# SegoleneMartin/transductive-CLIP

Measured on AMD Instinct MI355X. Metric: transductive tasks/sec (75-query EM-Dirichlet), higher is better.
Workload: dtype f32

## Files before the change

### include/tclip.h

```cpp
#ifndef TCLIP_H
#define TCLIP_H

#include <stddef.h>
#include <stdint.h>

#ifdef __cplusplus
extern "C" {
#endif

#define TCLIP_ABI_VERSION 5

enum {
    TCLIP_OK = 0,
    TCLIP_ERR_ARG = 1,
    TCLIP_ERR_WORKSPACE = 2,
    TCLIP_ERR_HIP = 3,
    TCLIP_ERR_INDEX = 4
};

typedef struct tclip_problem {
    int32_t n_batches;
    int32_t tasks_per_batch;
    int32_t n_query;
    int32_t n_class;
// ... 53 lines not shown
int tclip_em_gaussian_run(const tclip_problem* p, const float* x_q, float temperature, float* u, float* v, float* w,
                          int32_t* preds, void* workspace, size_t workspace_bytes, void* stream);

int tclip_em_gaussian_cov_run(const tclip_problem* p, const float* x_q, float* u, float* v, float* w, float* s,
                              int32_t* preds, void* workspace, size_t workspace_bytes, void* stream);

size_t tclip_hard_kmeans_workspace_bytes(const tclip_problem* p);
int tclip_hard_kmeans_run(const tclip_problem* p, const float* x_q, float* u, float* w, int32_t* preds,
                          float* criterions, void* workspace, size_t workspace_bytes, void* stream);

int tclip_kl_kmeans_run(const tclip_problem* p, const float* x_q, float* u, float* w, int32_t* preds,
                        float* criterions, void* workspace, size_t workspace_bytes, void* stream);

size_t tclip_bdcspn_workspace_bytes(const tclip_problem* p);
int tclip_bdcspn_run(const tclip_problem* p, const float* x_q, const float* x_s, const int64_t* y_s, float temp,
                     int32_t norm_type, float* prototypes, float* u, int32_t* preds, void* workspace,
                     size_t workspace_bytes, void* stream);

size_t tclip_paddle_workspace_bytes(const tclip_problem* p);
int tclip_paddle_run(const tclip_problem* p, const float* x_q, const float* x_s, const int64_t* y_s, float lambd,
                     float* u, float* v, float* w, int32_t* preds, void* workspace, size_t workspace_bytes,
                     void* stream);

#define TCLIP_TIM_SHANNON 0
#define TCLIP_TIM_ALPHA 1
typedef struct tclip_tim_params {
    double lr;
    float temp;
    float alpha_value;
    float loss_weights[3];
    int32_t entropies[3];
} tclip_tim_params;
size_t tclip_alpha_tim_workspace_bytes(const tclip_problem* p);
int tclip_alpha_tim_run(const tclip_problem* p, const tclip_tim_params* prm, const float* x_q, const float* x_s,
                        const int64_t* y_s, float* weights, float* logits_q, int32_t* preds, float* criterions,
                        void* workspace, size_t workspace_bytes, void* stream);

size_t tclip_laplacian_shot_workspace_bytes(const tclip_problem* p);
int tclip_laplacian_shot_run(const tclip_problem* p, const float* x_q, const float* x_s, const int64_t* y_s, int32_t knn,
                             double lmd, int32_t norm_type, float* unary, int32_t* neighbours, int32_t* preds_iter,
                             double* energies, void* workspace, size_t workspace_bytes, void* stream);

int tclip_argmax_rows(const float* x, int64_t n_rows, int32_t n_class, int32_t* labels, void* stream);

int tclip_probability_features(const float* visual, const float* text, int64_t n_rows, int32_t dim, int32_t n_class,
                               float temperature, float* out, void* stream);

int tclip_profile_enable(int on);
int tclip_profile_collect(double* mm_busy_ms, double* mm_launch_ms_sum, int64_t* mm_launches,
                          int64_t* element_updates);
int tclip_profile_last_kernels(double* busy_ms, double* launch_ms_sum, int64_t* launches, int64_t* element_updates);
int tclip_profile_last_split_sorts(int64_t* wave_iterations, int64_t* sorts);
int tclip_debug_set_split_keep_placement(int32_t on);

int tclip_debug_set_probe_chunks(int32_t chunks);

int tclip_debug_set_dead_head(int32_t iterations);

int tclip_debug_set_rowset_min_rows(int32_t rows);

int tclip_debug_set_mm_split(int32_t mode);

int tclip_debug_set_fixed_k_kernels(int32_t on);

int tclip_debug_set_kmeans_tile(int32_t mode);

int tclip_selftest_primitives(uint64_t* mismatches);

#ifdef __cplusplus
}
#endif
#endif
```

### transductive-clip_amd/csrc/tclip_kernels.hip

```cpp
#include <hip/hip_runtime.h>
#include <stdint.h>
#include <stdio.h>
#include <stdlib.h>
#include <string.h>

#include <algorithm>
#include <mutex>
#include <utility>
#include <vector>

#include "../../include/tclip.h"
#include "tclip_device.h"
#include "tclip_pk.h"
#include "tclip_selftest_inputs.h"

namespace tclip {

constexpr int kG64MinK = 897;

__global__ void k_log_features(const float* __restrict__ x, float* __restrict__ out, size_t n, int32_t* __restrict__ nonfinite) {
    bool bad = false;
    for (size_t i = (size_t)blockIdx.x * blockDim.x + threadIdx.x; i < n; i += (size_t)gridDim.x * blockDim.x) {
        const float v = log_f32(x[i] + kEpsF);
        out[i] = v;
// ... 262 lines not shown
        }
    }
    for (; i < Q; ++i) {
        const float fv = ft[(size_t)i * K];
#pragma unroll
        for (int j = 0; j < kMstatsRows; j++) a0[j] += term(j, ut[(size_t)i * K + j], fv);
    }
#pragma unroll
    for (int j = 0; j < kMstatsRows; j++) {
        const size_t row = (size_t)t * K + k0 + j;
        if (!live[row]) continue;
        float s = a0[j];
        s += a1[j];
        s += a2[j];
        s += a3[j];
        const float c = cs[row];
        if (kCov) {
            y[row * K + d] = c / (s < kEpsF ? kEpsF : s);
        } else if (paddle == 2) {
            y[row * K + d] = s / c;
        } else if (sup && paddle) {
            y[row * K + d] = (s + sup[row * K + d]) / (c + cnt[row]);
        } else if (sup) {
            const float w = 1.0f / (cnt[row] + c);
            y[row * K + d] = w * (sup[row * K + d] + s);
        } else {
            y[row * K + d] = s / (c < kEpsF ? kEpsF : c);
        }
    }
}

__device__ __forceinline__ int lanes_below_mask(unsigned long long m, int lane) { return __popcll(m & ((1ull << lane) - 1ull)); }

__global__ void k_build_rows(const uint8_t* __restrict__ live, const int32_t* __restrict__ cache_len, int n_rows,
                             int n_checks, int32_t* __restrict__ dead_rows, int32_t* __restrict__ live_rows,
                             int32_t* __restrict__ n_dead, int32_t* __restrict__ n_live) {
    const int i = blockIdx.x * blockDim.x + threadIdx.x;
    const bool in = i < n_rows;
    const bool alive = in && live[i];
    const bool need = in && !alive && n_checks > 0 && cache_len[i] < n_checks;
    const unsigned long long ml = __ballot(alive), md = __ballot(need);
    const int lane64 = threadIdx.x & 63;
    int base_l = 0, base_d = 0;
    if (lane64 == 0) {
        if (ml) base_l = atomicAdd(n_live, __popcll(ml));
        if (md) base_d = atomicAdd(n_dead, __popcll(md));
    }
    base_l = __shfl(base_l, 0, 64);
    base_d = __shfl(base_d, 0, 64);
    if (alive) live_rows[base_l + lanes_below_mask(ml, lane64)] = i;
    if (need) dead_rows[base_d + lanes_below_mask(md, lane64)] = i;
}

struct MMArgs {
    float* alpha;
    float* beta_dead;
    const float* y;
    const uint8_t* live;
    int32_t* cache_len;
    double* cache;
    double* rowpart;
    const int32_t* rows;
    const int32_t* n_rows;
    const int32_t* stop;
    unsigned long long* work_counter;
    int32_t* next_rows;
    int32_t* next_count;
    int K, rows_per_batch, chunk, l0, l1, has_check, n_checks;
    int keep_placement;
};

constexpr int kYRegsMaxE = 16;
template <int E, int G>
__device__ __forceinline__ int elem_of(int e, int lane) {
    if constexpr (G == 64) return (lane >> 5) * (E * 32) + e * 32 + (lane & 31);
    else return e * G + lane;
}
template <int E, int G>
__host__ __device__ constexpr int full_registers(int K) {
    if constexpr (G == 64) return K > E * 32 ? (K - E * 32) / 32 : 0;
    else return K / G;
}

template <int E, int G = kGroup, int kRegsMaxE = kYRegsMaxE>
struct RowY {
    static constexpr bool kInRegs = E <= kRegsMaxE;
    float r[kInRegs ? E : 1];
    const float* g;
    int lane, K, n_full;
    __device__ __forceinline__ void load(const float* row_y, int lane_, int K_) {
        g = row_y; lane = lane_; K = K_; n_full = full_registers<E, G>(K_);
        if (kInRegs) {
#pragma unroll
            for (int e = 0; e < (kInRegs ? E : 1); e++) {
                const int d = elem_of<E, G>(e, lane);
                r[e] = d < K ? (g ? g[d] : -10.0f) : 0.0f;
            }
        }
    }
    __device__ __forceinline__ void fetch_all(float (&out)[E]) const {
        if (!g) {
#pragma unroll
            for (int e = 0; e < E; e++) out[e] = -10.0f;
            return;
        }
        if constexpr (G == 64) {
            const float* base = g;
            asm volatile("" : "+s"(base));
            const __amdgpu_buffer_rsrc_t rsrc = __builtin_amdgcn_make_buffer_rsrc((void*)base, 0, K * 4, 0x00020000);
            int voff = elem_of<E, G>(0, lane) * 4;
            asm volatile("" : "+v"(voff));
#pragma unroll
            for (int e = 0; e < E; e++) out[e] = __builtin_bit_cast(float, __builtin_amdgcn_raw_buffer_load_b32(rsrc, voff + e * 128, 0, 0));
        } else {
#pragma unroll
            for (int e = 0; e < E; e++) out[e] = get(e);
        }
    }
    __device__ __forceinline__ float get(int e) const {
        if (kInRegs) return r[kInRegs ? e : 0];
// ... 447 lines not shown
        for (int w = 1; w < W; w++) at += j >= before[w] ? 64 * E * R - (before[w] - before[w - 1]) : 0;
        const float v = j < n_big ? queue[at] : 8.0f;
        const float r = lgamma_big_dense(v);
        if (j < n_big) queue[at] = r;
    }
    if (wave == (W - (turn % W) + 1) % W && lane64 < kGroups * R)
        ctl->psi[turn & 1][lane64] = digamma_pos_f32(ctl->rowsum[turn & 1][lane64], tab);
    __syncthreads();
    if (base[R] == 0) {
#pragma unroll
        for (int r = 0; r < R; r++)
            if (active[r])
                mm_apply_updates_small<E, G>(beta[r], yv[r], K, lane, ctl->psi[turn & 1][r * kGroups + (threadIdx.x / G)], tab,
                                             measure, num[r], den[r]);
        return;
    }
#pragma unroll
    for (int r = 0; r < R; r++)
        if (active[r])
            mm_apply_updates<E, G>(beta[r], yv[r], K, lane, ctl->psi[turn & 1][r * kGroups + (threadIdx.x / G)], tab, slice, base[r],
                                   measure, num[r], den[r]);
}

template <int E, int W, bool kDead, int R, int G = kGroup, int KC = 0>
__global__ __launch_bounds__(64 * W, (E > 16 ? kMMWavesLarge : kMMWavesSmall)) void k_mm_live(MMArgs a) {
    __shared__ LogTabEntry tab[16];
    __shared__ float queue[64 * W * E * R];
    __shared__ QueueCtl ctl;
    if (threadIdx.x == 0) ctl.bad = 0;
    load_log_table(tab);
    const int lane = threadIdx.x & (G - 1);
    const int group = threadIdx.x / G;
    constexpr int kGroups = (64 / G) * W, kRows = kGroups * R;
    static_assert(kRows <= 64, "QueueCtl holds 64 row sums");
    int turn = 0;
    const int n = *a.n_rows;
    const int K = KC > 0 ? KC : a.K;
    for (int first = blockIdx.x * kRows; first < n; first += gridDim.x * kRows) {
        int row[R];
        bool active[R];
        bool any = false;
#pragma unroll
        for (int r = 0; r < R; r++) {
            const int i = first + r * kGroups + group;
            row[r] = i < n ? a.rows[i] : 0;
            if constexpr (G == 64) row[r] = __builtin_amdgcn_readfirstlane(row[r]);
            const bool running = i < n && !a.stop[row[r] / a.rows_per_batch];
            const int have = (kDead && running) ? a.cache_len[row[r]] : 0;
            active[r] = running && (!kDead || have == a.chunk);
            any = any || active[r];
            if (kDead && a.next_rows && running && have < a.n_checks && lane == 0)
                a.next_rows[atomicAdd(a.next_count, 1)] = row[r];
        }
        if (!__syncthreads_or(any)) continue;
        const float* src = (kDead && a.chunk > 0) ? a.beta_dead : a.alpha;
        float* dst = kDead ? a.beta_dead : a.alpha;
        float beta[R][E];
        RowY<E, G> yv[R];
        double num[R], den[R];
#pragma unroll
        for (int r = 0; r < R; r++) {
            yv[r].load(kDead ? nullptr : a.y + (size_t)row[r] * K, lane, K);
#pragma unroll
            for (int e = 0; e < E; e++) {
                const int d = elem_of<E, G>(e, lane);
                beta[r][e] = (active[r] && d < K) ? src[(size_t)row[r] * K + d] : 0.0f;
            }
            num[r] = den[r] = 0.0;
        }
        for (int l = a.l0; l <= a.l1; l++)
            mm_iterate_block<E, W, R, G, KC>(beta, yv, K, lane, active, tab, queue, &ctl, turn++, a.has_check && l == a.l1, num, den);
#pragma unroll
        for (int r = 0; r < R; r++) {
            if (!active[r]) continue;
#pragma unroll
            for (int e = 0; e < E; e++) {
                const int d = elem_of<E, G>(e, lane);
                if (d < K) dst[(size_t)row[r] * K + d] = beta[r][e];
            }
            if (a.work_counter && lane == 0)
                atomicAdd(a.work_counter, (unsigned long long)K * (unsigned long long)(a.l1 - a.l0 + 1));
            if (a.has_check) {
                const double sn = group_sum_f64_g<G>(num[r]), sd = group_sum_f64_g<G>(den[r]);
                if (lane == 0) {
                    double* out = kDead ? a.cache + ((size_t)row[r] * a.n_checks + a.chunk) * 2 : a.rowpart + 2 * (size_t)row[r];
                    out[0] = sn;
                    out[1] = sd;
                    if (kDead) a.cache_len[row[r]] = a.chunk + 1;
                }
            }
        }
    }
}

constexpr int kSplitFrom = 1;
constexpr int kSplitMaxE = 24;
constexpr int kSplitYRegsMaxE = 8;
constexpr int kSplitMinE = 5;

__device__ __forceinline__ float lgamma_gt7_dense(float v) {
    bool sure;
    float r = lgamma_sleef_gt7_f64<true>(v, sure);
    if (__builtin_expect(__ballot(!sure) != 0ull, 0)) r = sure ? r : lgamma_sleef_ge23<true>(v);
    return r;
}

template <int E, int G, bool kTiny, bool kMeasure>
__device__ __forceinline__ void split_apply_updates(float (&beta)[E], const RowY<E, G, kSplitYRegsMaxE>& yv, int K, int lane, float psi_s,
                                                    const float* my0, const float* my1, const uint32_t (&slot)[(E + 1) / 2],
                                                    double& num, double& den) {
    constexpr bool measure = kMeasure;
    constexpr bool kYLocal = !RowY<E, G, kSplitYRegsMaxE>::kInRegs;
    float yl[kYLocal ? E : 1];
    if constexpr (kYLocal) yv.fetch_all(yl);
    auto y_of = [&](int e) { if constexpr (kYLocal) return yl[e]; else return yv.get(e); };
    const int n_full = full_registers<E, G>(K);
    auto finish = [&](int p, const PkUpdateStage& st) {
        const int e = 2 * p;
        const f2 a{beta[e], beta[e + 1]};
        const f2 nb = pk_mm_update_stage2(st);
        const bool full = e + 1 < n_full;
        const bool ok0 = full || elem_of<E, G>(e, lane) < K, ok1 = full || elem_of<E, G>(e + 1, lane) < K;
        if (measure) {
            const double d0 = (double)nb.x - (double)a.x, d1 = (double)nb.y - (double)a.y;
// ... 1343 lines not shown
    }
    for (uint32_t m = tid; m < (1u << 24); m += nth) {
        const float x = bits_f32(0x3f800000u + m);
        const f2 r = pk_sqrt_torch_inrange(f2{x, x * 0x1p-60f});
        b4 += f32_bits(r.x) != f32_bits(sqrt_torch_inrange_f32(x)) || f32_bits(r.y) != f32_bits(sqrt_torch_inrange_f32(x * 0x1p-60f));
        b4 += f32_bits(sqrt_torch_inrange_dev(x * 0x1p61f)) != f32_bits(sqrt_torch_inrange_f32(x * 0x1p61f));
    }
    for (int e = -100 + (int)tid; e <= 100; e += (int)nth) {
        const float x = bits_f32((uint32_t)(127 + e) << 23);
        b4 += f32_bits(sqrt_torch_inrange_dev(x)) != f32_bits(sqrt_torch_inrange_f32(x));
        b4 += f32_bits(pk_sqrt_torch_inrange(pk(x)).y) != f32_bits(sqrt_torch_inrange_f32(x));
    }
    atomicAdd(&out[0], b0); atomicAdd(&out[1], b1); atomicAdd(&out[2], b2);
    atomicAdd(&out[3], b3); atomicAdd(&out[4], b4); atomicAdd(&out[5], b5);
    for (int f = 0; f < kSelfTestFunctions; f++) {
        unsigned long long c = 0;
        for (uint32_t i = tid; i < kSelfTestCount; i += nth) c += selftest_term(f, i, tab);
        atomicAdd(&out[6 + f], c);
    }
}

thread_local char g_err[512] = "";

static int fail(int code, const char* fmt, const char* detail = "") {
    snprintf(g_err, sizeof g_err, fmt, detail);
    return code;
}

#define TCLIP_HIP(call)                                                                     \
    do {                                                                                    \
        hipError_t e_ = (call);                                                             \
        if (e_ != hipSuccess) return fail(TCLIP_ERR_HIP, #call ": %s", hipGetErrorString(e_)); \
    } while (0)

static size_t align_up(size_t x) { return (x + 255) & ~(size_t)255; }

struct Profile {
    bool on = false;
    std::vector<hipEvent_t> ev;
    std::vector<uint8_t> kind;
    size_t used = 0;
    unsigned long long* counter = nullptr;
    double last_busy[2] = {0, 0}, last_sum[2] = {0, 0};
    int64_t last_launches[2] = {0, 0}, last_updates[2] = {0, 0};
    int64_t last_split_iterations = 0, last_split_sorts = 0;
};
static thread_local bool g_last_mm_was_split = false;
thread_local Profile g_prof;
static int g_probe_chunks = kProbeChunks;
static int g_dead_head = kDeadHead;
static int g_rowset_min_rows = -1;
static int g_mm_split = -1;
static int g_split_keep_placement = 1;

static hipEvent_t prof_event() {
    if (g_prof.used == g_prof.ev.size()) {
        hipEvent_t e;
        if (hipEventCreate(&e) != hipSuccess) return nullptr;
        g_prof.ev.push_back(e);
    }
    return g_prof.ev[g_prof.used++];
}

constexpr int kDecideSlices = 64;
struct Layout {
    size_t logz, y, alpha_old, beta_dead, sup, cnt, cs, live, rowc, logit0, cache, cache_len, rowpart, mm_rows,
        mm_rows2, mm_rows3, dead_counts, cls, n_live, live_rows, counts, flags, stop, ratio, dpart, total;
    int n_checks;
};

static int n_chunks_of(int iter_mm) { return iter_mm <= 51 ? 1 : 1 + (iter_mm - 51 + 49) / 50; }
static int n_checks_of(int iter_mm) { return iter_mm <= 50 ? 0 : (iter_mm - 1) / 50; }

static Layout make_layout(const tclip_problem& p) {
    Layout L;
    const size_t T = (size_t)p.n_batches * p.tasks_per_batch, K = p.n_class, Q = p.n_query;
    const bool zs = p.n_support == 0;
    L.n_checks = n_checks_of(p.iter_mm);
    size_t o = 0;
    auto take = [&](size_t bytes) { size_t r = o; o += align_up(bytes); return r; };
    L.logz = take(T * Q * K * 4);
    L.y = take(T * K * K * 4);
    L.alpha_old = take(T * K * K * 4);
    L.beta_dead = take(zs ? T * K * K * 4 : 0);
    L.sup = take(zs ? 0 : T * K * K * 4);
    L.cnt = take(zs ? 0 : T * K * 4);
    L.cs = take(T * K * 4);
    L.live = take(T * K);
    L.rowc = take(T * K * 4);
    L.logit0 = take(T * Q * K * 4);
    L.cache = take(zs ? T * K * (size_t)L.n_checks * 16 : 0);
    L.cache_len = take(T * K * 4);
    L.rowpart = take(T * K * 16);
    L.mm_rows = take(T * K * 4);
    L.mm_rows2 = take(zs ? T * K * 4 : 0);
    L.mm_rows3 = take(zs ? T * K * 4 : 0);
    L.dead_counts = take(((size_t)n_chunks_of(p.iter_mm) + 3) * 4);
    L.cls = take(zs ? T * K * 2 : 0);
    L.n_live = take(zs ? T * 4 : 0);
    L.live_rows = take(T * K * 4);
    L.counts = take(256);
    L.flags = take(256);
    L.stop = take((size_t)p.n_batches * 4);
    L.ratio = take(T * 4);
    L.dpart = take((size_t)p.n_batches * kDecideSlices * 2 * sizeof(double));
    L.total = o;
    return L;
}

static int check_problem(const tclip_problem* p) {
    if (!p) return fail(TCLIP_ERR_ARG, "problem is null");
    if (p->n_batches < 1 || p->tasks_per_batch < 1 || p->n_query < 1 || p->iters < 0 || p->iter_mm < 1 ||
        p->n_support < 0)
        return fail(TCLIP_ERR_ARG, "non-positive size in tclip_problem");
    if (p->n_class < 2 || p->n_class > 1024) return fail(TCLIP_ERR_ARG, "n_class must be in 2..1024");
    if (p->n_support > 16000) return fail(TCLIP_ERR_ARG, "n_support must be <= 16000 (member lists are staged in LDS)");
    if ((long long)p->n_batches * p->tasks_per_batch > 65535) return fail(TCLIP_ERR_ARG, "n_batches*tasks_per_batch must be <= 65535 per call");
    if ((size_t)p->n_batches * p->tasks_per_batch * p->n_class > 0x7fffffffu)
        return fail(TCLIP_ERR_ARG, "n_batches*tasks_per_batch*n_class must fit in int32");
    return TCLIP_OK;
}

template <template <int> class Launcher, typename... Args>
static void dispatch_E(int K, Args... args) {
    const int need = (K + kGroup - 1) / kGroup;
    if (need <= 1) Launcher<1>::run(args...);
    else if (need <= 2) Launcher<2>::run(args...);
    else if (need <= 3) Launcher<3>::run(args...);
    else if (need <= 4) Launcher<4>::run(args...);
    else if (need <= 6) Launcher<6>::run(args...);
    else if (need <= 8) Launcher<8>::run(args...);
    else if (need <= 10) Launcher<10>::run(args...);
    else if (need <= 13) Launcher<13>::run(args...);
    else if (need <= 16) Launcher<16>::run(args...);
    else if (need <= 20) Launcher<20>::run(args...);
    else if (need <= 24) Launcher<24>::run(args...);
    else if (need <= 28) Launcher<28>::run(args...);
    else Launcher<32>::run(args...);
}

constexpr int kG16MaxK = 256;
static_assert(kG16MaxK >= 100 && kG16MaxK < 397 && kG64MinK <= 1000,
              "launch_mm's fixed-K kernels: K = 100 in the 16-lane, 397 in the 32-lane, 1000 in the 64-lane layout");
static int mm_lanes_per_row(int K) {
    if (g_rowset_min_rows == 0) return 32;
    if (K >= kG64MinK) return 64;
    return K <= kG16MaxK ? 16 : 32;
}
enum MMKind { kMMLive = 0, kMMDead = 1, kMMProbe = 2, kMMSplit = 3, kMMProbeHead = 4 };
template <int E, int G, int KC = 0>
static void launch_mm_EG(int dead, int rows, hipStream_t st, const MMArgs& a) {
    constexpr int kWaves = 4, kRowsPerBlock = (64 / G) * kWaves;
    int grid = (rows + kRowsPerBlock - 1) / kRowsPerBlock;
// ... 470 lines not shown
                          int16_t* cls = nullptr, int32_t* n_live = nullptr) {
    launch_mstats_mode<false>(st, u, f, cs, live, sup, cnt, T, Q, K, y, paddle, nullptr, dense, cls, n_live);
}
static void launch_cov_stats(hipStream_t st, const float* u, const float* z, const float* cs, const uint8_t* live,
                             const float* w, int T, int Q, int K, float* s) {
    launch_mstats_mode<true>(st, u, z, cs, live, nullptr, nullptr, T, Q, K, s, 0, w);
}

static int ew_grid(size_t n) {
    size_t g = (n + 255) / 256;
    return (int)(g > 8192 ? 8192 : (g < 1 ? 1 : g));
}

}

using namespace tclip;

extern "C" {

int tclip_abi_version(void) { return TCLIP_ABI_VERSION; }
const char* tclip_last_error(void) { return g_err; }

}

namespace tclip {

static int enqueue_batches(const tclip_problem& p, const RowSrc& q_src, const RowSrc& s_src, const int64_t* y_s, float* u,
                           float* v, float* alpha, int32_t* preds, float* criterions, int32_t* mm_iters,
                           char* ws, hipStream_t st) {
    const bool zs = p.n_support == 0;
    const Layout L = make_layout(p);
    const int B = p.n_batches, N = p.tasks_per_batch, Q = p.n_query, K = p.n_class, S = p.n_support;
    const int T = B * N, TK = T * K;
    const size_t TQK = (size_t)T * Q * K, TKK = (size_t)T * K * K;
    float* logz = (float*)(ws + L.logz);
    float* y = (float*)(ws + L.y);
    float* alpha_old = (float*)(ws + L.alpha_old);
    float* beta_dead = zs ? (float*)(ws + L.beta_dead) : nullptr;
    float* sup = zs ? nullptr : (float*)(ws + L.sup);
    float* cnt = zs ? nullptr : (float*)(ws + L.cnt);
    float* cs = (float*)(ws + L.cs);
    uint8_t* live = (uint8_t*)(ws + L.live);
    float* rowc = (float*)(ws + L.rowc);
    float* logit0 = (float*)(ws + L.logit0);
    double* cache = zs ? (double*)(ws + L.cache) : nullptr;
    int32_t* cache_len = (int32_t*)(ws + L.cache_len);
    double* rowpart = (double*)(ws + L.rowpart);
    int32_t* mm_rows = (int32_t*)(ws + L.mm_rows);
    int32_t* dead_list[2] = {mm_rows, zs ? (int32_t*)(ws + L.mm_rows2) : mm_rows};
    int32_t* dead_counts = (int32_t*)(ws + L.dead_counts);
    int32_t* head_back = zs ? (int32_t*)(ws + L.mm_rows3) : nullptr;
    int32_t* live_rows = (int32_t*)(ws + L.live_rows);
    int32_t* counts = (int32_t*)(ws + L.counts);
    int32_t* flags = (int32_t*)(ws + L.flags);
    int32_t* stop = (int32_t*)(ws + L.stop);
    float* ratio = (float*)(ws + L.ratio);
    double* dpart = (double*)(ws + L.dpart);
    const int n_chunks = n_chunks_of(p.iter_mm);
    const int n_checks = zs ? L.n_checks : 0;

    TCLIP_HIP(hipMemsetAsync(flags, 0, 256, st));
    if (q_src.idx) {
        const size_t rows = (size_t)T * Q;
        hipLaunchKernelGGL(k_gather_log_features, dim3((unsigned)(rows > 65536 ? 65536 : rows)), dim3(256), 0, st, q_src, Q, K, rows, u, logz, flags);
    } else {
        hipLaunchKernelGGL(k_log_features, dim3(ew_grid(TQK)), dim3(256), 0, st, q_src.base, logz, TQK, flags);
        hipLaunchKernelGGL(k_copy, dim3(ew_grid(TQK)), dim3(256), 0, st, q_src.base, u, TQK);
    }
    hipLaunchKernelGGL(k_fill, dim3(ew_grid(TKK)), dim3(256), 0, st, alpha, 1.0f, TKK);
    hipLaunchKernelGGL(k_fill, dim3(ew_grid(TKK)), dim3(256), 0, st, alpha_old, 1.0f, TKK);
    hipLaunchKernelGGL(k_fill, dim3(ew_grid(TK)), dim3(256), 0, st, v, 0.0f, (size_t)TK);
    TCLIP_HIP(hipMemsetAsync(cache_len, 0, (size_t)TK * 4, st));
    if (!zs) {
        hipLaunchKernelGGL(k_support_stats, dim3(K, T), dim3(128), (size_t)S * sizeof(int), st, s_src, y_s, S, K, 1, sup, cnt);
    }
    {
        TCLIP_HIP(hipMemsetAsync(counts, 0, 256, st));
        hipLaunchKernelGGL(k_one_row_list, dim3(1), dim3(1), 0, st, mm_rows, counts + 2);
        dispatch_E<LaunchRowConsts>(K, 1, st, (const float*)alpha, (const int32_t*)mm_rows, (const int32_t*)(counts + 2), K, rowc);
        hipLaunchKernelGGL(k_broadcast_first, dim3(ew_grid((size_t)TK)), dim3(256), 0, st, rowc, (size_t)TK);
        TCLIP_HIP(hipMemsetAsync(live, 1, (size_t)TK, st));
        hipLaunchKernelGGL(k_build_rows, dim3((TK + 255) / 256), dim3(256), 0, st, live, cache_len, TK, 0, mm_rows,
                           live_rows, counts, counts + 1);
        hipLaunchKernelGGL(k_init_logits, dim3(ew_grid(TQK)), dim3(256), 0, st, (const float*)rowc, (const int32_t*)flags, Q, K, TQK, logit0);
        dispatch_E<LaunchLogits>(K, TK > 262144 ? 262144 : TK, st, (const float*)alpha, (const float*)logz, (const float*)rowc,
                                 (const int32_t*)live_rows, (const int32_t*)(counts + 1), Q, K, logit0, (const int32_t*)flags);
    }

    for (int it = 0; it < p.iters; it++) {
        hipLaunchKernelGGL(k_cluster_sizes, dim3((TK + 255) / 256), dim3(256), 0, st, (const float*)u, T, Q, K, zs ? 1 : 0,
                           cs, live, v, cache_len);
        launch_mstats(st, (const float*)u, (const float*)logz, (const float*)cs, (const uint8_t*)live, (const float*)sup, (const float*)cnt, T, Q, K, y, 0,
                      !zs || it == 0, (zs && it > 0) ? (int16_t*)(ws + L.cls) : nullptr, (zs && it > 0) ? (int32_t*)(ws + L.n_live) : nullptr);
        TCLIP_HIP(hipMemsetAsync(counts, 0, 256, st));
        TCLIP_HIP(hipMemsetAsync(dead_counts, 0, ((size_t)n_chunks + 3) * 4, st));
        TCLIP_HIP(hipMemsetAsync(stop, 0, (size_t)B * 4, st));
        hipLaunchKernelGGL(k_build_rows, dim3((TK + 255) / 256), dim3(256), 0, st, (const uint8_t*)live,
                           (const int32_t*)cache_len, TK, n_checks, dead_list[0], live_rows, dead_counts, counts + 1);
        for (int c = 0; c < n_chunks; c++) {
            MMArgs a;
            a.alpha = alpha; a.beta_dead = beta_dead; a.y = y; a.live = live; a.cache_len = cache_len;
            a.cache = cache; a.rowpart = rowpart; a.rows = mm_rows; a.n_rows = counts; a.stop = stop;
            a.next_rows = nullptr; a.next_count = nullptr;
            a.K = K; a.rows_per_batch = N * K; a.chunk = c;
            a.keep_placement = g_split_keep_placement;
            a.l0 = c == 0 ? 0 : 50 * c + 1;
            a.l1 = 50 * (c + 1) < p.iter_mm - 1 ? 50 * (c + 1) : p.iter_mm - 1;
            a.has_check = (a.l1 > 0 && a.l1 % 50 == 0) ? 1 : 0;
            a.n_checks = n_checks > 0 ? n_checks : 1;
            const bool split = g_mm_split < 0 ? it >= kSplitFrom : (g_mm_split >= 100 ? it >= g_mm_split - 100 : g_mm_split != 0);
            const bool split_runs = split && mm_has_split(K);
            a.work_counter = g_prof.on ? g_prof.counter + (split_runs ? 1 : 0) : nullptr;
            hipEvent_t e0 = g_prof.on ? prof_event() : nullptr, e1 = g_prof.on ? prof_event() : nullptr;
            if (e0 && e1) TCLIP_HIP(hipEventRecord(e0, st));
            a.rows = live_rows; a.n_rows = counts + 1;
            g_last_mm_was_split = false;
            launch_mm(split ? kMMSplit : kMMLive, K, TK, st, a);
            if (e0 && e1) {
                TCLIP_HIP(hipEventRecord(e1, st));
                if (g_prof.kind.size() < g_prof.used / 2) g_prof.kind.resize(g_prof.used / 2);
                g_prof.kind[g_prof.used / 2 - 1] = g_last_mm_was_split ? 1 : 0;
            }
            if (split_runs != g_last_mm_was_split) return fail(TCLIP_ERR_ARG, "internal: mm_has_split disagrees with launch_mm");
            if (zs && a.has_check) {
                a.rows = dead_list[c & 1]; a.n_rows = dead_counts + c; a.work_counter = nullptr;
                if (c == 0 && g_dead_head > 0 && g_probe_chunks > 0) {
                    MMArgs h = a;
                    h.l0 = 0; h.l1 = g_dead_head - 1; h.has_check = 0; h.next_rows = nullptr; h.next_count = nullptr;
                    launch_mm(kMMDead, K, TK, st, h);
                    h.l0 = g_dead_head; h.next_rows = head_back; h.next_count = dead_counts + n_chunks + 2;
                    launch_mm(kMMProbeHead, K, TK, st, h);
                    a.rows = head_back; a.n_rows = dead_counts + n_chunks + 2;
                }
                const bool more = c + 1 < a.n_checks, probe = c < g_probe_chunks && more;
                int32_t* next_rows = more ? dead_list[(c + 1) & 1] : nullptr;
                int32_t* next_count = more ? dead_counts + c + 1 : nullptr;
                a.next_rows = probe ? nullptr : next_rows; a.next_count = probe ? nullptr : next_count;
                launch_mm(kMMDead, K, TK, st, a);
                a.next_rows = next_rows; a.next_count = next_count;
                if (probe) launch_mm(kMMProbe, K, TK, st, a);
            }
            const bool two_stage = a.has_check && N * K > 16384;
            if (two_stage)
                hipLaunchKernelGGL(k_mm_decide_partial, dim3(kDecideSlices, B), dim3(256), 0, st, (const double*)rowpart,
                                   (const double*)cache, (const uint8_t*)live, N * K, a.n_checks, c, (const int32_t*)stop, dpart);
            hipLaunchKernelGGL(k_mm_decide, dim3(B), dim3(1024), 0, st, (const double*)rowpart, (const double*)cache,
                               (const uint8_t*)live, N * K, a.n_checks, c, a.has_check, a.l1, c == n_chunks - 1 ? 1 : 0,
                               p.iter_mm, stop, mm_iters + it, p.iters, (const double*)(two_stage ? dpart : nullptr),
                               kDecideSlices);
        }
        {
            const int g8 = (TK + 7) / 8 > 65535 * 8 ? 65535 * 8 : (TK + 7) / 8;
            dispatch_E<LaunchRowConsts>(K, g8 > 4096 ? 4096 : g8, st, (const float*)alpha, (const int32_t*)live_rows,
                                        (const int32_t*)(counts + 1), K, rowc);
            dispatch_E<LaunchLogits>(K, TK > kLogitsGrid ? kLogitsGrid : TK, st, (const float*)alpha, (const float*)logz, (const float*)rowc,
                                     (const int32_t*)live_rows, (const int32_t*)(counts + 1), Q, K, logit0, (const int32_t*)nullptr);
        }
        hipLaunchKernelGGL(k_softmax, dim3((T * Q * 16 + 255) / 256), dim3(256), 0, st, (const float*)logit0, (const float*)v,
                           T * Q, Q, K, (float)p.lambd, p.hard, 0, u, preds);
        hipLaunchKernelGGL(k_criterion, dim3(T), dim3(64), 0, st, (const float*)alpha, alpha_old, K, T, ratio);
        hipLaunchKernelGGL(k_criterion_mean, dim3(B), dim3(64), 0, st, (const float*)ratio, N, (!zs && p.hard) ? 1 : 0,
                           criterions + it, p.iters);
    }
    TCLIP_HIP(hipGetLastError());
    return TCLIP_OK;
}

constexpr int kMaxGroups = 16;
struct StreamPool {
    hipStream_t s[kMaxGroups] = {};
    hipEvent_t fork = nullptr, join[kMaxGroups] = {};
    bool ready = false;
    int device = -1;
};
thread_local StreamPool g_pool;

static int pool_init(int groups) {
    int dev = 0;
    TCLIP_HIP(hipGetDevice(&dev));
    if (g_pool.ready && g_pool.device != dev) {
        for (int i = 0; i < kMaxGroups; i++) {
            if (g_pool.s[i]) (void)hipStreamDestroy(g_pool.s[i]);
            if (g_pool.join[i]) (void)hipEventDestroy(g_pool.join[i]);
            g_pool.s[i] = nullptr;
            g_pool.join[i] = nullptr;
        }
        (void)hipEventDestroy(g_pool.fork);
        g_pool.fork = nullptr;
        g_pool.ready = false;
    }
    g_pool.device = dev;
    if (!g_pool.fork) TCLIP_HIP(hipEventCreateWithFlags(&g_pool.fork, hipEventDisableTiming));
    for (int i = 1; i < groups && i < kMaxGroups; i++) {
        if (g_pool.s[i]) continue;
        TCLIP_HIP(hipStreamCreateWithFlags(&g_pool.s[i], hipStreamNonBlocking));
        TCLIP_HIP(hipEventCreateWithFlags(&g_pool.join[i], hipEventDisableTiming));
    }
    g_pool.ready = true;
    return TCLIP_OK;
}

static int stream_groups() {
    static const int n = [] {
        const char* e = getenv("TCLIP_STREAM_GROUPS");
        const int v = e ? atoi(e) : 3;
        return v < 1 ? 1 : (v > kMaxGroups ? kMaxGroups : v);
    }();
    return n;
}
// ... 473 lines not shown
                               (size_t)kKmeansTile * stride * sizeof(float), st, (const float*)w, x_q, Q, K, stride, divs);
        } else {
            dispatch_E<LaunchKlDivergences>(K, T, st, (const float*)w, x_q, Q, K, divs);
        }
        hipLaunchKernelGGL(k_argmin_rows, dim3((T * Q + 255) / 256), dim3(256), 0, st, (const float*)divs, T * Q, K, preds);
        hipLaunchKernelGGL(k_hard_assign, dim3(T), dim3(256), 0, st, (const int32_t*)preds, Q, K, u, change);
        hipLaunchKernelGGL(k_criterion_mean, dim3(B), dim3(64), 0, st, (const float*)change, N, 0, criterions + it, p.iters);
    }
    TCLIP_HIP(hipGetLastError());
    return TCLIP_OK;
}

int tclip_argmax_rows(const float* x, int64_t n_rows, int32_t n_class, int32_t* labels, void* stream) {
    if (!x || !labels || n_rows < 0 || n_class < 1) return fail(TCLIP_ERR_ARG, "bad argument to tclip_argmax_rows");
    if (n_rows == 0) return TCLIP_OK;
    hipLaunchKernelGGL(k_argmax_rows, dim3((unsigned)((n_rows + 255) / 256)), dim3(256), 0, (hipStream_t)stream, x, (long)n_rows,
                       n_class, labels);
    TCLIP_HIP(hipGetLastError());
    return TCLIP_OK;
}

int tclip_probability_features(const float* visual, const float* text, int64_t n_rows, int32_t dim, int32_t n_class,
                               float temperature, float* out, void* stream) {
    if (!visual || !text || !out || n_rows < 0 || dim < 1 || n_class < 1) return fail(TCLIP_ERR_ARG, "bad argument to tclip_probability_features");
    if (n_rows == 0) return TCLIP_OK;
    const size_t lds = ((size_t)dim + (size_t)n_class) * sizeof(float);
    if (lds > 60000 || n_rows > 0x7fffffff) return fail(TCLIP_ERR_ARG, "dim + n_class must be <= 15000");
    hipLaunchKernelGGL(k_probability_features, dim3((unsigned)n_rows), dim3(256), lds, (hipStream_t)stream, visual, text,
                       dim, n_class, temperature, out);
    TCLIP_HIP(hipGetLastError());
    return TCLIP_OK;
}

int tclip_debug_set_rowset_min_rows(int32_t rows) {
    g_rowset_min_rows = rows;
    return TCLIP_OK;
}

int tclip_debug_set_kmeans_tile(int32_t mode) {
    g_kmeans_tile = mode;
    return TCLIP_OK;
}

int tclip_debug_set_fixed_k_kernels(int32_t on) {
    g_fixed_k_kernels = on;
    return TCLIP_OK;
}

int tclip_debug_set_mm_split(int32_t mode) {
    g_mm_split = mode;
    return TCLIP_OK;
}

int tclip_debug_set_split_keep_placement(int32_t on) {
    g_split_keep_placement = on != 0;
    return TCLIP_OK;
}

int tclip_debug_set_dead_head(int32_t iterations) {
    if (iterations > 18) return fail(TCLIP_ERR_ARG, "tclip_debug_set_dead_head: at most 18 iterations");
    g_dead_head = iterations < 0 ? kDeadHead : iterations;
    return TCLIP_OK;
}
int tclip_debug_set_probe_chunks(int32_t chunks) {
    g_probe_chunks = chunks < 0 ? kProbeChunks : chunks;
    return TCLIP_OK;
}

int tclip_profile_enable(int on) {
    if (on && !g_prof.counter) {
        TCLIP_HIP(hipMalloc((void**)&g_prof.counter, 4 * sizeof(unsigned long long)));
        TCLIP_HIP(hipMemset(g_prof.counter, 0, 4 * sizeof(unsigned long long)));
    }
    g_prof.on = on != 0;
    return TCLIP_OK;
}

static double union_ms(std::vector<std::pair<float, float>>& iv) {
    std::sort(iv.begin(), iv.end());
    double busy = 0.0, cur_lo = 0.0, cur_hi = -1.0;
    for (auto& x : iv) {
        if (cur_hi < cur_lo || x.first > cur_hi) {
            if (cur_hi >= cur_lo) busy += cur_hi - cur_lo;
            cur_lo = x.first;
            cur_hi = x.second;
        } else if (x.second > cur_hi) {
            cur_hi = x.second;
        }
    }
    if (cur_hi >= cur_lo) busy += cur_hi - cur_lo;
    return busy;
}
int tclip_profile_collect(double* mm_busy_ms, double* mm_launch_ms_sum, int64_t* mm_launches,
                          int64_t* element_updates) {
    TCLIP_HIP(hipDeviceSynchronize());
    std::vector<std::pair<float, float>> iv, ivk[2];
    double sum = 0.0;
    for (int k = 0; k < 2; k++) { g_prof.last_sum[k] = 0.0; g_prof.last_launches[k] = 0; }
    for (size_t i = 0; i + 1 < g_prof.used; i += 2) {
        float t0 = 0.f, t1 = 0.f;
        TCLIP_HIP(hipEventElapsedTime(&t0, g_prof.ev[0], g_prof.ev[i]));
        TCLIP_HIP(hipEventElapsedTime(&t1, g_prof.ev[0], g_prof.ev[i + 1]));
        iv.emplace_back(t0, t1);
        sum += (double)t1 - (double)t0;
        const int k = i / 2 < g_prof.kind.size() ? g_prof.kind[i / 2] : 0;
        ivk[k].emplace_back(t0, t1);
// ... 122 lines not shown
```

### transductive-clip_amd/tclip_amd/_capi.py

```python
import ctypes
import os

_HERE = os.path.dirname(os.path.abspath(__file__))
LIB_PATH = os.path.join(_HERE, "libtclip.so")


class Problem(ctypes.Structure):
    _fields_ = [(n, ctypes.c_int32) for n in (
        "n_batches", "tasks_per_batch", "n_query", "n_class", "n_support", "iters", "iter_mm", "lambd", "hard")]


class TaskSource(ctypes.Structure):
    _fields_ = [(n, ctypes.c_void_p) for n in ("table_q", "q_idx", "table_s", "s_idx", "cols")]


class TimParams(ctypes.Structure):
    _fields_ = [("lr", ctypes.c_double), ("temp", ctypes.c_float), ("alpha_value", ctypes.c_float),
                ("loss_weights", ctypes.c_float * 3), ("entropies", ctypes.c_int32 * 3)]


_P = ctypes.c_void_p
_SIGNATURES = {
    "tclip_abi_version": (ctypes.c_int, []),
    "tclip_last_error": (ctypes.c_char_p, []),
    "tclip_workspace_bytes": (ctypes.c_size_t, [ctypes.POINTER(Problem)]),
    "tclip_em_dirichlet_run": (ctypes.c_int, [ctypes.POINTER(Problem)] + [_P] * 10 + [ctypes.c_size_t, _P]),
    "tclip_em_dirichlet_run_tasks": (ctypes.c_int, [ctypes.POINTER(Problem), ctypes.POINTER(TaskSource)] + [_P] * 8 + [ctypes.c_size_t, _P]),
    "tclip_prototype_workspace_bytes": (ctypes.c_size_t, [ctypes.c_int32] * 3),
    "tclip_cluster_prototypes": (ctypes.c_int, [ctypes.c_int32] * 3 + [_P] * 6 + [ctypes.c_size_t, _P]),
    "tclip_match_clusters_host": (ctypes.c_int, [ctypes.c_int32] * 3 + [_P] * 5 + [ctypes.c_int32, _P, _P]),
    "tclip_match_clusters_host_strided": (ctypes.c_int, [ctypes.c_int32] * 3 + [_P] * 5 + [ctypes.c_int32, ctypes.c_int32, _P, _P]),
    "tclip_host_threads": (ctypes.c_int, []),
    "tclip_gather_rows": (ctypes.c_int, [_P, ctypes.c_int64, ctypes.c_int32, _P, ctypes.c_int64, _P, _P]),
    "tclip_soft_kmeans_workspace_bytes": (ctypes.c_size_t, [ctypes.POINTER(Problem)]),
    "tclip_soft_kmeans_run": (ctypes.c_int, [ctypes.POINTER(Problem), _P, ctypes.c_float, _P, _P, _P, _P, ctypes.c_size_t, _P]),
    "tclip_em_gaussian_run": (ctypes.c_int, [ctypes.POINTER(Problem), _P, ctypes.c_float, _P, _P, _P, _P, _P, ctypes.c_size_t, _P]),
    "tclip_em_gaussian_cov_run": (ctypes.c_int, [ctypes.POINTER(Problem), _P, _P, _P, _P, _P, _P, _P, ctypes.c_size_t, _P]),
    "tclip_paddle_workspace_bytes": (ctypes.c_size_t, [ctypes.POINTER(Problem)]),
    "tclip_paddle_run": (ctypes.c_int, [ctypes.POINTER(Problem), _P, _P, _P, ctypes.c_float, _P, _P, _P, _P, _P, ctypes.c_size_t, _P]),
    "tclip_alpha_tim_workspace_bytes": (ctypes.c_size_t, [ctypes.POINTER(Problem)]),
    "tclip_alpha_tim_run": (ctypes.c_int, [ctypes.POINTER(Problem), ctypes.POINTER(TimParams)] + [_P] * 8 + [ctypes.c_size_t, _P]),
    "tclip_laplacian_shot_workspace_bytes": (ctypes.c_size_t, [ctypes.POINTER(Problem)]),
    "tclip_laplacian_shot_run": (ctypes.c_int, [ctypes.POINTER(Problem), _P, _P, _P, ctypes.c_int32, ctypes.c_double, ctypes.c_int32,
                                                _P, _P, _P, _P, _P, ctypes.c_size_t, _P]),
    "tclip_bdcspn_workspace_bytes": (ctypes.c_size_t, [ctypes.POINTER(Problem)]),
    "tclip_bdcspn_run": (ctypes.c_int, [ctypes.POINTER(Problem), _P, _P, _P, ctypes.c_float, ctypes.c_int32, _P, _P, _P, _P, ctypes.c_size_t, _P]),
    "tclip_hard_kmeans_workspace_bytes": (ctypes.c_size_t, [ctypes.POINTER(Problem)]),
    "tclip_hard_kmeans_run": (ctypes.c_int, [ctypes.POINTER(Problem), _P, _P, _P, _P, _P, _P, ctypes.c_size_t, _P]),
    "tclip_kl_kmeans_run": (ctypes.c_int, [ctypes.POINTER(Problem), _P, _P, _P, _P, _P, _P, ctypes.c_size_t, _P]),
    "tclip_argmax_rows": (ctypes.c_int, [_P, ctypes.c_int64, ctypes.c_int32, _P, _P]),
    "tclip_probability_features": (ctypes.c_int, [_P, _P, ctypes.c_int64, ctypes.c_int32, ctypes.c_int32, ctypes.c_float, _P, _P]),
    "tclip_selftest_primitives": (ctypes.c_int, [ctypes.POINTER(ctypes.c_uint64)]),
    "tclip_profile_enable": (ctypes.c_int, [ctypes.c_int]),
    "tclip_debug_set_probe_chunks": (ctypes.c_int, [ctypes.c_int32]),
    "tclip_debug_set_dead_head": (ctypes.c_int, [ctypes.c_int32]),
    "tclip_debug_set_rowset_min_rows": (ctypes.c_int, [ctypes.c_int32]),
    "tclip_debug_set_mm_split": (ctypes.c_int, [ctypes.c_int32]),
    "tclip_debug_set_split_keep_placement": (ctypes.c_int, [ctypes.c_int32]),
    "tclip_debug_set_fixed_k_kernels": (ctypes.c_int, [ctypes.c_int32]),
    "tclip_debug_set_kmeans_tile": (ctypes.c_int, [ctypes.c_int32]),
    "tclip_profile_last_kernels": (ctypes.c_int, [ctypes.POINTER(ctypes.c_double), ctypes.POINTER(ctypes.c_double),
                                                  ctypes.POINTER(ctypes.c_int64), ctypes.POINTER(ctypes.c_int64)]),
    "tclip_check_task_indices": (ctypes.c_int, [_P, ctypes.c_int64, ctypes.c_int64, _P, ctypes.c_int64, ctypes.c_int32, _P]),
    "tclip_profile_last_split_sorts": (ctypes.c_int, [ctypes.POINTER(ctypes.c_int64), ctypes.POINTER(ctypes.c_int64)]),
    "tclip_profile_collect": (ctypes.c_int, [ctypes.POINTER(ctypes.c_double), ctypes.POINTER(ctypes.c_double),
                                             ctypes.POINTER(ctypes.c_int64), ctypes.POINTER(ctypes.c_int64)]),
}
EXPORTS = tuple(_SIGNATURES)
_lib = None


def lib():
    global _lib
    if _lib is None:
        path = os.environ.get("TCLIP_LIB") or LIB_PATH
        if not os.path.exists(path):
            raise RuntimeError(
                f"{path} is missing: build it with `python transductive-clip_amd/build.py` "
                "(there is no CPU or PyTorch fallback for the EM-Dirichlet path)")
        import torch
        hip_rt = os.path.join(os.path.dirname(torch.__file__), "lib", "libamdhip64.so")
        if os.path.exists(hip_rt):
            ctypes.CDLL(hip_rt, mode=ctypes.RTLD_GLOBAL)
        l = ctypes.CDLL(path)
        for name, (res, args) in _SIGNATURES.items():
            fn = getattr(l, name)
            fn.restype, fn.argtypes = res, args
        if l.tclip_abi_version() != 5:
            raise RuntimeError("libtclip.so ABI version mismatch")
        _lib = l
    return _lib


def _strip_comments(text):
    out, i, n = [], 0, len(text)
    while i < n:
        c = text[i]
        if c == '"' or c == "'":
            j = i + 1
            while j < n and text[j] != c:
                j += 2 if text[j] == "\\" else 1
            out.append(text[i:j + 1])
            i = j + 1
        elif text.startswith("//", i):
            j = text.find("\n", i)
            i = n if j < 0 else j
        elif text.startswith("/*", i):
            j = text.find("*/", i + 2)
            i = n if j < 0 else j + 2
        else:
            out.append(c)
# ... 20 lines not shown
```

### transductive-clip_amd/tclip_amd/engine.py

```python
import ctypes

import torch

from . import _capi


def _ptr(t):
    return ctypes.c_void_p(t.data_ptr()) if t is not None else None


def _stream():
    return ctypes.c_void_p(torch.cuda.current_stream().cuda_stream)


def _require_cuda(t, name):
    if not t.is_cuda:
        raise RuntimeError(f"{name} must live on the GPU: the EM-Dirichlet engine has no CPU path")


class EMDirichletResult:
    __slots__ = ("u", "v", "alpha", "preds", "criterions", "mm_iters")

    def __init__(self, **kw):
        for k, val in kw.items():
# ... 242 lines not shown
    dev = x_q.device
    lib = _capi.lib()
    cmax = min(Q, K)
    with torch.cuda.device(dev):
        ws_bytes = lib.tclip_prototype_workspace_bytes(T, Q, K)
        ws = torch.empty(ws_bytes + 256, dtype=torch.uint8, device=dev)
        off = (-ws.data_ptr()) % 256
        n_clusters = torch.empty(T, dtype=torch.int32, device=dev)
        ids = torch.empty(T, cmax, dtype=torch.int32, device=dev)
        protos = torch.empty(T, cmax, K, device=dev)
        preds = preds.to(dev).int().contiguous()
        rc = lib.tclip_cluster_prototypes(T, Q, K, _ptr(x_q), _ptr(preds), _ptr(n_clusters), _ptr(ids), _ptr(protos),
                                          ctypes.c_void_p(ws.data_ptr() + off), ws_bytes, _stream())
        _capi.check(rc, "tclip_cluster_prototypes")
        preds_h, nc_h = preds.cpu(), n_clusters.cpu()
        used = max(1, min(cmax, int(nc_h.max())))
        ids_h = torch.empty((T, used), dtype=torch.int32, pin_memory=True)
        protos_h = torch.empty((T, used, K), dtype=torch.float32, pin_memory=True)
        ids_h.copy_(ids[:, :used], non_blocking=True)
        protos_h.copy_(protos[:, :used], non_blocking=True)
        torch.cuda.current_stream().synchronize()
    y_h = y_q.reshape(T, Q).long().cpu().contiguous()
    new_preds = torch.empty(T, Q, dtype=torch.int32)
    acc = torch.empty(T, dtype=torch.float32)
    rc = lib.tclip_match_clusters_host_strided(T, Q, K, _ptr(preds_h), _ptr(nc_h), _ptr(ids_h), _ptr(protos_h), _ptr(y_h),
                                               int(bool(graph_matching)), used, _ptr(new_preds), _ptr(acc))
    _capi.check(rc, "tclip_match_clusters_host_strided")
    return acc, new_preds


def gather_rows(table, idx):
    _require_cuda(table, "table")
    table = table.contiguous().float()
    idx = _index_tensor(idx.reshape(-1), table.shape[0], table.device, "idx")
    out = torch.empty(idx.numel(), table.shape[1], device=table.device)
    with torch.cuda.device(table.device):
        rc = _capi.lib().tclip_gather_rows(_ptr(table), table.shape[0], table.shape[1], _ptr(idx), idx.numel(), _ptr(out), _stream())
    _capi.check(rc, "tclip_gather_rows")
    return out


def debug_set_probe_chunks(chunks=-1):
    _capi.check(_capi.lib().tclip_debug_set_probe_chunks(int(chunks)), "tclip_debug_set_probe_chunks")


def debug_set_dead_head(iterations=-1):
    _capi.check(_capi.lib().tclip_debug_set_dead_head(int(iterations)), "tclip_debug_set_dead_head")


def debug_set_rowset_min_rows(rows=-1):
    _capi.check(_capi.lib().tclip_debug_set_rowset_min_rows(int(rows)), "tclip_debug_set_rowset_min_rows")


def profile_enable(on=True):
    _capi.check(_capi.lib().tclip_profile_enable(int(bool(on))), "tclip_profile_enable")


def profile_collect():
    busy, total, n, upd = ctypes.c_double(0), ctypes.c_double(0), ctypes.c_int64(0), ctypes.c_int64(0)
    _capi.check(_capi.lib().tclip_profile_collect(ctypes.byref(busy), ctypes.byref(total), ctypes.byref(n),
                                                  ctypes.byref(upd)), "tclip_profile_collect")
    return busy.value, total.value, n.value, upd.value


def profile_last_kernels():
    busy, total = (ctypes.c_double * 2)(), (ctypes.c_double * 2)()
    n, upd = (ctypes.c_int64 * 2)(), (ctypes.c_int64 * 2)()
    _capi.check(_capi.lib().tclip_profile_last_kernels(busy, total, n, upd), "tclip_profile_last_kernels")
    return {name: (busy[i], total[i], n[i], upd[i]) for i, name in enumerate(("k_mm_live", "k_mm_split"))}


def profile_last_split_sorts():
    it, so = ctypes.c_int64(0), ctypes.c_int64(0)
    _capi.check(_capi.lib().tclip_profile_last_split_sorts(ctypes.byref(it), ctypes.byref(so)), "tclip_profile_last_split_sorts")
    return it.value, so.value
```

Before: 168.5.

## Partition live MM rows by small-beta flag between chunks

During each non-final MM chunk, the live kernel now flags rows whose Dirichlet parameters all stay below a threshold, or rows that did no work. After the chunk, a two-kernel stable partition (block counts, then a ballot-based scatter) reorders the live row list so flagged and unflagged rows are grouped. The goal is to make work per wave more uniform and cut divergence or tail imbalance in later chunks. The cost is two extra launches per chunk, a per-row byte write, and a second row buffer in the workspace. A debug mode can turn this off or reverse the order.

```diff
diff --git a/include/tclip.h b/include/tclip.h
--- a/include/tclip.h
+++ b/include/tclip.h
@@ -129,6 +129,7 @@
 int tclip_profile_last_kernels(double* busy_ms, double* launch_ms_sum, int64_t* launches, int64_t* element_updates);
 int tclip_profile_last_split_sorts(int64_t* wave_iterations, int64_t* sorts);
 int tclip_debug_set_split_keep_placement(int32_t on);
+int tclip_debug_set_live_row_order(int32_t mode);
 
 int tclip_debug_set_probe_chunks(int32_t chunks);
 
diff --git a/transductive-clip_amd/csrc/tclip_kernels.hip b/transductive-clip_amd/csrc/tclip_kernels.hip
--- a/transductive-clip_amd/csrc/tclip_kernels.hip
+++ b/transductive-clip_amd/csrc/tclip_kernels.hip
@@ -338,6 +338,60 @@
     if (need) dead_rows[base_d + lanes_below_mask(md, lane64)] = i;
 }
 
+constexpr int kPartBlocks = 256;
+__device__ __forceinline__ int block_sum_256(int v, int* red) {
+    for (int m = 32; m >= 1; m >>= 1) v += __shfl_xor(v, m, 64);
+    __syncthreads();
+    if ((threadIdx.x & 63) == 0) red[threadIdx.x >> 6] = v;
+    __syncthreads();
+    return red[0] + red[1] + red[2] + red[3];
+}
+__global__ __launch_bounds__(kPartBlocks) void k_partition_count(const int32_t* __restrict__ rows, const int32_t* __restrict__ n_rows,
+                                                                 const uint8_t* __restrict__ flag, int32_t* __restrict__ part) {
+    __shared__ int red[4];
+    const int n = *n_rows, tile = (n + kPartBlocks - 1) / kPartBlocks;
+    const int b0 = blockIdx.x * tile, b1 = min(n, b0 + tile);
+    int c = 0;
+    if (flag)
+        for (int i = b0 + (int)threadIdx.x; i < b1; i += kPartBlocks) c += flag[rows[i]] != 0;
+    c = block_sum_256(c, red);
+    if (threadIdx.x == 0) part[blockIdx.x] = c;
+}
+__global__ __launch_bounds__(kPartBlocks) void k_partition_scatter(const int32_t* __restrict__ rows, const int32_t* __restrict__ n_rows,
+                                                                   const uint8_t* __restrict__ flag, const int32_t* __restrict__ part,
+                                                                   int32_t* __restrict__ out, int reverse) {
+    __shared__ int red[4], wf[4], wu[4];
+    const int n = *n_rows, tile = (n + kPartBlocks - 1) / kPartBlocks;
+    const int b0 = blockIdx.x * tile, b1 = min(n, b0 + tile);
+    const int total = block_sum_256(part[threadIdx.x], red);
+    int f = block_sum_256((int)threadIdx.x < (int)blockIdx.x ? part[threadIdx.x] : 0, red);
+    int u = total + (b0 - f);
+    const int wave = threadIdx.x >> 6;
+    for (int base = b0; base < b1; base += kPartBlocks) {
+        const int i = base + (int)threadIdx.x;
+        const bool in = i < b1;
+        const int r = in ? rows[i] : 0;
+        const bool fl = in && flag && flag[r] != 0;
+        const unsigned long long mf = __ballot(fl), mu = __ballot(in && !fl);
+        if ((threadIdx.x & 63) == 0) {
+            wf[wave] = __popcll(mf);
+            wu[wave] = __popcll(mu);
+        }
+        __syncthreads();
+        int bf = 0, bu = 0;
+        for (int w = 0; w < wave; w++) {
+            bf += wf[w];
+            bu += wu[w];
+        }
+        const int lane64 = threadIdx.x & 63;
+        const int p = fl ? f + bf + lanes_below_mask(mf, lane64) : u + bu + lanes_below_mask(mu, lane64);
+        if (in) out[reverse ? n - 1 - p : p] = r;
+        f += wf[0] + wf[1] + wf[2] + wf[3];
+        u += wu[0] + wu[1] + wu[2] + wu[3];
+        __syncthreads();
+    }
+}
+
 struct MMArgs {
     float* alpha;
     float* beta_dead;
@@ -352,6 +406,7 @@
     unsigned long long* work_counter;
     int32_t* next_rows;
     int32_t* next_count;
+    uint8_t* small;
     int K, rows_per_batch, chunk, l0, l1, has_check, n_checks;
     int keep_placement;
 };
@@ -905,7 +960,14 @@
             if (kDead && a.next_rows && running && have < a.n_checks && lane == 0)
                 a.next_rows[atomicAdd(a.next_count, 1)] = row[r];
         }
-        if (!__syncthreads_or(any)) continue;
+        if (!__syncthreads_or(any)) {
+            if (!kDead && a.small && lane == 0) {
+#pragma unroll
+                for (int r = 0; r < R; r++)
+                    if (first + r * kGroups + group < n) a.small[row[r]] = 1;
+            }
+            continue;
+        }
         const float* src = (kDead && a.chunk > 0) ? a.beta_dead : a.alpha;
         float* dst = kDead ? a.beta_dead : a.alpha;
         float beta[R][E];
@@ -923,6 +985,17 @@
         }
         for (int l = a.l0; l <= a.l1; l++)
             mm_iterate_block<E, W, R, G, KC>(beta, yv, K, lane, active, tab, queue, &ctl, turn++, a.has_check && l == a.l1, num, den);
+        if (!kDead && a.small) {
+#pragma unroll
+            for (int r = 0; r < R; r++) {
+                bool big = false;
+#pragma unroll
+                for (int e = 0; e < E; e++) big = big || (active[r] && beta[r][e] + 1.0f >= 2.3f);
+                const unsigned long long m = __builtin_amdgcn_ballot_w64(big);
+                const unsigned long long mine = G == 64 ? m : (m >> ((threadIdx.x & 63) & ~(G - 1))) & ((1ull << (G & 63)) - 1ull);
+                if (lane == 0 && first + r * kGroups + group < n) a.small[row[r]] = mine == 0ull;
+            }
+        }
 #pragma unroll
         for (int r = 0; r < R; r++) {
             if (!active[r]) continue;
@@ -2372,6 +2445,7 @@
 static int g_rowset_min_rows = -1;
 static int g_mm_split = -1;
 static int g_split_keep_placement = 1;
+static int g_live_row_order = 0;
 
 static hipEvent_t prof_event() {
     if (g_prof.used == g_prof.ev.size()) {
@@ -2385,7 +2459,7 @@
 constexpr int kDecideSlices = 64;
 struct Layout {
     size_t logz, y, alpha_old, beta_dead, sup, cnt, cs, live, rowc, logit0, cache, cache_len, rowpart, mm_rows,
-        mm_rows2, mm_rows3, dead_counts, cls, n_live, live_rows, counts, flags, stop, ratio, dpart, total;
+        mm_rows2, mm_rows3, dead_counts, cls, n_live, live_rows, live_rows2, row_small, part, counts, flags, stop, ratio, dpart, total;
     int n_checks;
 };
 
@@ -2419,6 +2493,9 @@
     L.cls = take(zs ? T * K * 2 : 0);
     L.n_live = take(zs ? T * 4 : 0);
     L.live_rows = take(T * K * 4);
+    L.live_rows2 = take(T * K * 4);
+    L.row_small = take(T * K);
+    L.part = take(kPartBlocks * 4);
     L.counts = take(256);
     L.flags = take(256);
     L.stop = take((size_t)p.n_batches * 4);
@@ -2995,6 +3072,16 @@
     int32_t* head_back = zs ? (int32_t*)(ws + L.mm_rows3) : nullptr;
     int32_t* live_rows = (int32_t*)(ws + L.live_rows);
     int32_t* counts = (int32_t*)(ws + L.counts);
+    int32_t* rows_cur = live_rows;
+    int32_t* rows_other = (int32_t*)(ws + L.live_rows2);
+    uint8_t* row_small = (uint8_t*)(ws + L.row_small);
+    auto partition_rows = [&](const uint8_t* flag) {
+        hipLaunchKernelGGL(k_partition_count, dim3(kPartBlocks), dim3(kPartBlocks), 0, st, (const int32_t*)rows_cur,
+                           (const int32_t*)(counts + 1), flag, (int32_t*)(ws + L.part));
+        hipLaunchKernelGGL(k_partition_scatter, dim3(kPartBlocks), dim3(kPartBlocks), 0, st, (const int32_t*)rows_cur,
+                           (const int32_t*)(counts + 1), flag, (const int32_t*)(ws + L.part), rows_other, g_live_row_order == 2 ? 1 : 0);
+        std::swap(rows_cur, rows_other);
+    };
     int32_t* flags = (int32_t*)(ws + L.flags);
     int32_t* stop = (int32_t*)(ws + L.stop);
     float* ratio = (float*)(ws + L.ratio);
@@ -3040,11 +3127,14 @@
         TCLIP_HIP(hipMemsetAsync(stop, 0, (size_t)B * 4, st));
         hipLaunchKernelGGL(k_build_rows, dim3((TK + 255) / 256), dim3(256), 0, st, (const uint8_t*)live,
                            (const int32_t*)cache_len, TK, n_checks, dead_list[0], live_rows, dead_counts, counts + 1);
+        rows_cur = live_rows;
+        rows_other = (int32_t*)(ws + L.live_rows2);
+        if (g_live_row_order == 2) partition_rows(nullptr);
         for (int c = 0; c < n_chunks; c++) {
             MMArgs a;
             a.alpha = alpha; a.beta_dead = beta_dead; a.y = y; a.live = live; a.cache_len = cache_len;
             a.cache = cache; a.rowpart = rowpart; a.rows = mm_rows; a.n_rows = counts; a.stop = stop;
-            a.next_rows = nullptr; a.next_count = nullptr;
+            a.next_rows = nullptr; a.next_count = nullptr; a.small = nullptr;
             a.K = K; a.rows_per_batch = N * K; a.chunk = c;
             a.keep_placement = g_split_keep_placement;
             a.l0 = c == 0 ? 0 : 50 * c + 1;
@@ -3056,7 +3146,9 @@
             a.work_counter = g_prof.on ? g_prof.counter + (split_runs ? 1 : 0) : nullptr;
             hipEvent_t e0 = g_prof.on ? prof_event() : nullptr, e1 = g_prof.on ? prof_event() : nullptr;
             if (e0 && e1) TCLIP_HIP(hipEventRecord(e0, st));
-            a.rows = live_rows; a.n_rows = counts + 1;
+            a.rows = rows_cur; a.n_rows = counts + 1;
+            const bool reorder = g_live_row_order != 1 && !split_runs && c + 1 < n_chunks;
+            if (reorder) a.small = row_small;
             g_last_mm_was_split = false;
             launch_mm(split ? kMMSplit : kMMLive, K, TK, st, a);
             if (e0 && e1) {
@@ -3066,7 +3158,7 @@
             }
             if (split_runs != g_last_mm_was_split) return fail(TCLIP_ERR_ARG, "internal: mm_has_split disagrees with launch_mm");
             if (zs && a.has_check) {
-                a.rows = dead_list[c & 1]; a.n_rows = dead_counts + c; a.work_counter = nullptr;
+                a.rows = dead_list[c & 1]; a.n_rows = dead_counts + c; a.work_counter = nullptr; a.small = nullptr;
                 if (c == 0 && g_dead_head > 0 && g_probe_chunks > 0) {
                     MMArgs h = a;
                     h.l0 = 0; h.l1 = g_dead_head - 1; h.has_check = 0; h.next_rows = nullptr; h.next_count = nullptr;
@@ -3091,13 +3183,15 @@
                                (const uint8_t*)live, N * K, a.n_checks, c, a.has_check, a.l1, c == n_chunks - 1 ? 1 : 0,
                                p.iter_mm, stop, mm_iters + it, p.iters, (const double*)(two_stage ? dpart : nullptr),
                                kDecideSlices);
+            if (reorder) partition_rows(row_small);
+            else if (g_live_row_order == 2 && c + 1 < n_chunks) partition_rows(nullptr);
         }
         {
             const int g8 = (TK + 7) / 8 > 65535 * 8 ? 65535 * 8 : (TK + 7) / 8;
-            dispatch_E<LaunchRowConsts>(K, g8 > 4096 ? 4096 : g8, st, (const float*)alpha, (const int32_t*)live_rows,
+            dispatch_E<LaunchRowConsts>(K, g8 > 4096 ? 4096 : g8, st, (const float*)alpha, (const int32_t*)rows_cur,
                                         (const int32_t*)(counts + 1), K, rowc);
             dispatch_E<LaunchLogits>(K, TK > kLogitsGrid ? kLogitsGrid : TK, st, (const float*)alpha, (const float*)logz, (const float*)rowc,
-                                     (const int32_t*)live_rows, (const int32_t*)(counts + 1), Q, K, logit0, (const int32_t*)nullptr);
+                                     (const int32_t*)rows_cur, (const int32_t*)(counts + 1), Q, K, logit0, (const int32_t*)nullptr);
         }
         hipLaunchKernelGGL(k_softmax, dim3((T * Q * 16 + 255) / 256), dim3(256), 0, st, (const float*)logit0, (const float*)v,
                            T * Q, Q, K, (float)p.lambd, p.hard, 0, u, preds);
@@ -3677,6 +3771,12 @@
     return TCLIP_OK;
 }
 
+int tclip_debug_set_live_row_order(int32_t mode) {
+    if (mode > 2) return fail(TCLIP_ERR_ARG, "tclip_debug_set_live_row_order: mode 0, 1 or 2");
+    g_live_row_order = mode < 0 ? 0 : mode;
+    return TCLIP_OK;
+}
+
 int tclip_debug_set_split_keep_placement(int32_t on) {
     g_split_keep_placement = on != 0;
     return TCLIP_OK;
diff --git a/transductive-clip_amd/tclip_amd/_capi.py b/transductive-clip_amd/tclip_amd/_capi.py
--- a/transductive-clip_amd/tclip_amd/_capi.py
+++ b/transductive-clip_amd/tclip_amd/_capi.py
@@ -57,6 +57,7 @@
     "tclip_debug_set_rowset_min_rows": (ctypes.c_int, [ctypes.c_int32]),
     "tclip_debug_set_mm_split": (ctypes.c_int, [ctypes.c_int32]),
     "tclip_debug_set_split_keep_placement": (ctypes.c_int, [ctypes.c_int32]),
+    "tclip_debug_set_live_row_order": (ctypes.c_int, [ctypes.c_int32]),
     "tclip_debug_set_fixed_k_kernels": (ctypes.c_int, [ctypes.c_int32]),
     "tclip_debug_set_kmeans_tile": (ctypes.c_int, [ctypes.c_int32]),
     "tclip_profile_last_kernels": (ctypes.c_int, [ctypes.POINTER(ctypes.c_double), ctypes.POINTER(ctypes.c_double),
diff --git a/transductive-clip_amd/tclip_amd/engine.py b/transductive-clip_amd/tclip_amd/engine.py
--- a/transductive-clip_amd/tclip_amd/engine.py
+++ b/transductive-clip_amd/tclip_amd/engine.py
@@ -318,6 +318,10 @@
     _capi.check(_capi.lib().tclip_debug_set_rowset_min_rows(int(rows)), "tclip_debug_set_rowset_min_rows")
 
 
+def debug_set_live_row_order(mode=-1):
+    _capi.check(_capi.lib().tclip_debug_set_live_row_order(int(mode)), "tclip_debug_set_live_row_order")
+
+
 def profile_enable(on=True):
     _capi.check(_capi.lib().tclip_profile_enable(int(bool(on))), "tclip_profile_enable")
 
```

Measured after the change: 169.3 (median of 6 runs). No clear change (+0.5%).
